# AlexGidiotis/Multimodal-Gesture-Recognition-with-LSTMs-and-CTC

Measured on AMD Instinct MI355X. Metric: train frames/sec, fusion BiLSTM+CTC, higher is better.
Workload: dtype f32

## Files before the change

multimodal-gesture-recognition-with-lstms-and-ctc_amd/csrc/gemm.hip:

```cpp
#include "common.h"
#include "split_f16.h"

namespace {

#ifndef MGR_GEMM_BK
#define MGR_GEMM_BK 16
#endif
#ifndef MGR_GEMM_NBUF
#define MGR_GEMM_NBUF 2
#endif
constexpr int BM = 128, BN = 128, BK = MGR_GEMM_BK, NBUF = MGR_GEMM_NBUF, LDS_LD = BM + 4;
constexpr int LPT = BK / 8;

struct RegTile {
  float v[4 * LPT];
};

__device__ __forceinline__ void load_kc(RegTile& r, const float* __restrict__ base, size_t ld, int m0, int k0, int Mlim,
                                        int Klim, bool vec, int tid) {
#pragma unroll
  for (int i = 0; i < LPT; ++i) {
    int idx4 = tid + i * 256;
    int m = idx4 / (BK / 4), k4 = (idx4 % (BK / 4)) * 4;
    int gm = m0 + m, gk = k0 + k4;
// ... 420 lines not shown
#pragma unroll
          for (int i = 0; i < APT; ++i) As[buf][ak & 3][ar + ARS * i][ak >> 2] = R.a[i];
        }
        *reinterpret_cast<float4*>(&Bs[buf][q][r][0]) = make_float4(R.w[0] * R.v[0], R.w[1] * R.v[1], R.w[2] * R.v[2], R.w[3] * R.v[3]);
      };
      auto mma = [&](int buf) {
        const int ra = wr * 64 + l31, ub = wc * 32 + l31;
        const f32x4 a00 = *reinterpret_cast<const f32x4*>(&As[buf][2 * lh][ra][0]);
        const f32x4 a01 = *reinterpret_cast<const f32x4*>(&As[buf][2 * lh + 1][ra][0]);
        const f32x4 a10 = *reinterpret_cast<const f32x4*>(&As[buf][2 * lh][ra + 32][0]);
        const f32x4 a11 = *reinterpret_cast<const f32x4*>(&As[buf][2 * lh + 1][ra + 32][0]);
        const f32x4 b0 = *reinterpret_cast<const f32x4*>(&Bs[buf][2 * lh][ub][0]);
        const f32x4 b1 = *reinterpret_cast<const f32x4*>(&Bs[buf][2 * lh + 1][ub][0]);
#pragma unroll
        for (int c = 0; c < 4; ++c) {
          acc[g][0] = __builtin_amdgcn_mfma_f32_32x32x2f32(a00[c], b0[c], acc[g][0], 0, 0, 0);
          acc[g][1] = __builtin_amdgcn_mfma_f32_32x32x2f32(a10[c], b0[c], acc[g][1], 0, 0, 0);
        }
#pragma unroll
        for (int c = 0; c < 4; ++c) {
          acc[g][0] = __builtin_amdgcn_mfma_f32_32x32x2f32(a01[c], b1[c], acc[g][0], 0, 0, 0);
          acc[g][1] = __builtin_amdgcn_mfma_f32_32x32x2f32(a11[c], b1[c], acc[g][1], 0, 0, 0);
        }
      };
      if (nst > 0) {
        Regs R0, R1;
        fetch(R0, 0);
        if (nst > 1) fetch(R1, 1);
        stash(R0, 0);
        __syncthreads();
        for (int st = 0; st < nst; st += 2) {
          if (st + 2 < nst) fetch(R0, st + 2);
          mma(0);
          if (st + 1 < nst) stash(R1, 1);
          __syncthreads();
          if (st + 1 < nst) {
            if (st + 3 < nst) fetch(R1, st + 3);
            mma(1);
            if (st + 2 < nst) stash(R0, 0);
            __syncthreads();
          }
        }
      }
    }
    const int unit = acc_col(u0 + wc * 32, l31);
    if (unit < H) {
      const float4 bias = *reinterpret_cast<const float4*>(bp + unit * 4);
      store_z_tile<true>(acc, 1.f, bias, Z, b, T, N, r0 + wr * 64, unit, lh);
    }
  }
}

constexpr int NP_MAXF = 64, NP_TU = 64, NP_RPW = 3;
static inline size_t np_lds_bytes(int F) { return ((size_t)SP_TM * (F | 1) + (size_t)4 * F * NP_TU) * sizeof(float); }

template <int XR>
__global__ __launch_bounds__(256, XR > 20 ? 1 : 2) void k_proj_narrow(const float* __restrict__ X, int ldx, const float* __restrict__ mask4,
                                                        const float* __restrict__ Wp, const float* __restrict__ bp, float* __restrict__ Z,
                                                        int B, int T, int F, int H) {
  constexpr int TM = SP_TM, TU = NP_TU;
  extern __shared__ __attribute__((aligned(16))) float np_lds[];
  __shared__ int Lf[4][NP_MAXF];
  __shared__ float Lv[4][NP_MAXF];
  __shared__ int Lc[4];
  const int pitch = F | 1;
  float* Xs = np_lds;
  float* Ws = np_lds + TM * pitch;
  const int tid = threadIdx.x, lane = tid & 63, wave = tid >> 6, wr = wave >> 1, wc = wave & 1;
  const int l31 = lane & 31, lh = lane >> 5;
  const int N = 4 * H;
  const int ncol = (H + TU - 1) / TU, nrow = (T + TM - 1) / TM, nchunk = (nrow + NP_RPW - 1) / NP_RPW;
  const XcdTile wt = xcd_tile(blockIdx.x, ncol);
  const int rc = wt.group;
  if (rc >= nchunk * B) return;
  const int u0 = wt.item * TU, b = rc / nchunk, rt0 = (rc % nchunk) * NP_RPW;
  const int rt1 = rt0 + NP_RPW < nrow ? rt0 + NP_RPW : nrow;
  {
    const int Fp = (F + SP_SK - 1) / SP_SK * SP_SK;
    const bool valid = lane < F;
    const float v = valid ? mask4[((size_t)wave * B + b) * F + lane] : 0.f;
    const bool kept = valid && v != 0.f;
    const unsigned long long kb = __ballot(kept), db = __ballot(valid && !kept), lower = (1ull << lane) - 1ull;
    const int cnt = __popcll(kb);
    if (valid) {
      const int pos = kept ? __popcll(kb & lower) : cnt + __popcll(db & lower);
      Lf[wave][pos] = lane;
      Lv[wave][pos] = v;
    } else if (lane < Fp) {
      Lf[wave][lane] = 0;
      Lv[wave][lane] = 0.f;
    }
    if (lane == 0) Lc[wave] = cnt;
  }
  {
    constexpr int WR = (XR + 1) / 2;
    float4 w[WR];
#pragma unroll
    for (int k = 0; k < WR; ++k) {
      const int i = tid + 256 * k < F * TU ? tid + 256 * k : F * TU - 1;
      const int f = i / TU, u = i % TU;
      const int uc = u0 + u < H ? u0 + u : H - 1;
      w[k] = *reinterpret_cast<const float4*>(Wp + (unsigned)((f * H + uc) * 4));
    }
#pragma unroll
    for (int k = 0; k < WR; ++k) {
      const int i = tid + 256 * k;
      if (i < F * TU) {
        const int f = i / TU, u = i % TU;
        Ws[(0 * F + f) * TU + u] = w[k].x;
        Ws[(1 * F + f) * TU + u] = w[k].y;
        Ws[(2 * F + f) * TU + u] = w[k].z;
        Ws[(3 * F + f) * TU + u] = w[k].w;
      }
    }
  }
  const int ra = wr * 64 + l31, ub = wc * 32 + l31;
  const int unit = u0 + ub;
  float4 bias = make_float4(0.f, 0.f, 0.f, 0.f);
  if (unit < H) bias = *reinterpret_cast<const float4*>(bp + unit * 4);
  const int dq = 256 / F, dr = 256 % F, row_0 = tid / F, col_0 = tid % F;
  const float* Xb = X + (size_t)b * T * ldx;
  float xv[XR];
  auto xload = [&](int rt) {
    int row = row_0, col = col_0;
#pragma unroll
    for (int k = 0; k < XR; ++k) {
      const int rw = row < TM ? row : TM - 1;
      const int rcl = rt * TM + rw < T ? rt * TM + rw : T - 1;
      xv[k] = Xb[(unsigned)(rcl * ldx + col)];
      row += dq;
      col += dr;
      if (col >= F) {
        col -= F;
        ++row;
      }
    }
  };
  xload(rt0);
  for (int rt = rt0; rt < rt1; ++rt) {
    const int r0 = rt * TM;
    __syncthreads();
    {
      int row = row_0, col = col_0;
#pragma unroll
      for (int k = 0; k < XR; ++k) {
        if (row < TM) Xs[row * pitch + col] = xv[k];
        row += dq;
        col += dr;
        if (col >= F) {
          col -= F;
          ++row;
        }
      }
    }
    __syncthreads();
    if (rt + 1 < rt1) xload(rt + 1);
    f32x16 acc[4][2];
    zero_acc(acc);
#pragma unroll
    for (int g = 0; g < 4; ++g) {
      const int nst = (Lc[g] + SP_SK - 1) / SP_SK;
      const float* Wsg = Ws + (size_t)g * F * TU + ub;
      const float* Xa = Xs + ra * pitch;
      for (int st = 0; st < nst; ++st) {
#pragma unroll
        for (int ks = 0; ks < 8; ++ks) {
          const int p = st * SP_SK + 2 * lh + (ks >> 2) + 4 * (ks & 3);
          const int f = Lf[g][p];
          const float bv = Wsg[f * TU] * Lv[g][p];
          acc[g][0] = __builtin_amdgcn_mfma_f32_32x32x2f32(Xa[f], bv, acc[g][0], 0, 0, 0);
          acc[g][1] = __builtin_amdgcn_mfma_f32_32x32x2f32(Xa[32 * pitch + f], bv, acc[g][1], 0, 0, 0);
        }
      }
    }
    if (unit < H) store_z_tile<true>(acc, 1.f, bias, Z, b, T, N, r0 + wr * 64, unit, lh);
  }
}

__global__ __launch_bounds__(256, 2) void k_gemm_nn_sparse16(const float* __restrict__ X, int ldx, const int* __restrict__ kidx,
                                                             const float* __restrict__ kval, const int* __restrict__ kcnt,
                                                             const float* __restrict__ Wp, const float* __restrict__ bp,
                                                             float* __restrict__ Z, int B, int T, int Fp, int F, int H,
                                                             const unsigned* __restrict__ wmax, float vmax, float sx, const unsigned* __restrict__ gate) {
  MGR_GATED(gate, false);
  constexpr int TM = SP_TM, TU = 64, SK = SP_SK, NT = 256, QT = 64, RPT = 2;
  __shared__ __attribute__((aligned(16))) _Float16 Ah[2][2][TM][8], Al[2][2][TM][8];
  __shared__ __attribute__((aligned(16))) _Float16 Bh[2][2][TU][8], Bl[2][2][TU][8];
  __shared__ unsigned short Ls[SP_MAXF];
  __shared__ float Vs[SP_MAXF];
  const int tid = threadIdx.x, lane = tid & 63, wave = tid >> 6, wr = wave >> 1, wc = wave & 1;
  const int N = 4 * H;
  const int q = tid / QT, r = tid % QT;
  const int l31 = lane & 31, lh = lane >> 5;
  const int ncol = (H + TU - 1) / TU, nrow = (T + TM - 1) / TM;
  const float sw = split_scale<SPLIT_NONFINITE_ZERO>(__uint_as_float(*wmax) * vmax, -60);
  const float inv = split_unscale(1.f, sw, sx);
  struct Regs {
    float a[RPT * 4], w[4], v[4];
  };
  const XcdTile wt = xcd_tile(blockIdx.x, ncol);
  const int rt = wt.group;
  if (rt >= nrow * B) return;
  const int u0 = wt.item * TU, r0 = (rt % nrow) * TM, b = rt / nrow;
  const float* Xb = X + (size_t)b * F * ldx + r0 + r;
  const int ucl = (u0 + r < H) ? u0 + r : H - 1;
  f32x16 acc[4][2];
  zero_acc(acc);
#pragma unroll
  for (int g = 0; g < 4; ++g) {
    const int nst1 = (kcnt[g * B + b] + SK - 1) / SK;
    const int nst = (nst1 + 1) & ~1;
    {
      const int* list = kidx + ((size_t)g * B + b) * Fp;
      const float* lval = kval + ((size_t)g * B + b) * Fp;
      for (int i = tid; i < nst * SK; i += NT) {
        const bool in = i < nst1 * SK;
        Ls[i] = in ? (unsigned short)list[i] : (unsigned short)0;
        Vs[i] = in ? lval[i] : 0.f;
      }
    }
    __syncthreads();
    const float* Wg = Wp + (size_t)g * F * H + ucl;
// ... 643 lines not shown
  const int Nd = 4 * H;
  const bool fast = (ldx % 4 == 0) && (F % BK == 0) && aligned16(X) && aligned16(Wp_fwd) && aligned16(Wp_rev);
  if (!fast || (2 * Nd + BN - 1) / BN >= 2 * ((Nd + BN - 1) / BN)) {
    int r = mgr_lstm_input_proj(c, X, ldx, mask4_fwd, Wp_fwd, bp_fwd, Z_fwd, B, T, F, H);
    if (r) return r;
    return mgr_lstm_input_proj(c, X, ldx, mask4_rev, Wp_rev, bp_rev, Z_rev, B, T, F, H);
  }
  dim3 grid((2 * Nd + BN - 1) / BN, (T + BM - 1) / BM, B);
  mgr_prof_begin(c, MGR_K_GEMM_NN);
  hipLaunchKernelGGL(k_gemm_nn2, grid, dim3(256), 0, mgr_stream(c), X, ldx, mask4_fwd, mask4_rev, Wp_fwd, Wp_rev, bp_fwd, bp_rev,
                     Z_fwd, Z_rev, B, T, F, Nd);
  MGR_LAUNCH_CHECK();
  mgr_prof_end(c, MGR_K_GEMM_NN);
  return 0;
}

static size_t sp_fp(int F) { return (size_t)(F + SP_SK - 1) / SP_SK * SP_SK; }

struct ProjDropWs { int* kidx; float* kval; int* kcnt; unsigned* wmax; float* Wg; size_t bytes; };
static ProjDropWs proj_dropout_ws_layout(void* ws, int B, int F, int H) {
  mgr_ws_carver w(ws);
  const size_t nl = (size_t)4 * B * sp_fp(F);
  return {w.take<int>(nl), w.take<float>(nl), w.take<int>((size_t)4 * B), w.take<unsigned>(64), w.take<float>((size_t)F * 4 * H), w.off};
}
size_t mgr_lstm_input_proj_dropout_ws_bytes(int B, int F, int H) { return proj_dropout_ws_layout(nullptr, B, F, H).bytes; }

static bool sparse_proj_shape(const mgr_ctx* c, float drop_rate, int F) {
  return drop_rate >= 0.3f && F >= 16 && F <= SP_MAXF && c->tune[MGR_TUNE_PROJ_DENSE] == 0;
}

int mgr_lstm_input_proj_dropout_wants_transposed(mgr_ctx* c, float drop_rate, int F) {
  return (c && sparse_proj_shape(c, drop_rate, F) && F >= 128) ? 1 : 0;
}

static int input_proj_dropout_impl(mgr_ctx* c, const float* X, int ldx, bool transposed, const float* mask4, float drop_rate,
                                   const float* Wp, const float* bp, float* Z, int B, int T, int F, int H, void* ws, size_t ws_bytes,
                                   float x_absmax = 0.f) {
  const int Fp = (int)sp_fp(F);
  const ProjDropWs L = proj_dropout_ws_layout(ws, B, F, H);
  int *kidx = L.kidx, *kcnt = L.kcnt;
  float *kval = L.kval, *Wg = L.Wg;
  unsigned* wmax = L.wmax;
  hipStream_t s = mgr_stream(c);
  const SplitCall sc = split_call(c, x_absmax, transposed && drop_rate < 0.99f, wmax + 1);
  const bool f16 = sc.f16;
  unsigned* const gate = sc.gate;
  const bool dense = f16 && (!mask4 || c->tune[MGR_TUNE_PROJ_DENSE16_MASKED] == 2);
  MGR_REQUIRE(mask4 || transposed, "a projection without a dropout mask is only handled from the transposed copy");
  const bool lists = !dense || gate;
  mgr_prof_begin(c, MGR_K_GEMM_NN);
  if (!transposed && mask4 && F >= 16 && F <= NP_MAXF && c->tune[MGR_TUNE_PROJ_WIDE_TILES] != 2) {
    if (!(c->attr_done & MGR_ATTR_PROJ_NARROW)) {
      MGR_HIP(hipFuncSetAttribute(reinterpret_cast<const void*>(k_proj_narrow<32>), hipFuncAttributeMaxDynamicSharedMemorySize, (int)np_lds_bytes(NP_MAXF)));
      c->attr_done |= MGR_ATTR_PROJ_NARROW;
    }
    const int nchunk = ((T + SP_TM - 1) / SP_TM + NP_RPW - 1) / NP_RPW;
    const int nwg = ((H + NP_TU - 1) / NP_TU) * ((nchunk * B + 7) / 8) * 8;
    if (F <= 20)
      hipLaunchKernelGGL(k_proj_narrow<10>, dim3(nwg), dim3(256), np_lds_bytes(F), s, X, ldx, mask4, Wp, bp, Z, B, T, F, H);
    else if (F <= 40)
      hipLaunchKernelGGL(k_proj_narrow<20>, dim3(nwg), dim3(256), np_lds_bytes(F), s, X, ldx, mask4, Wp, bp, Z, B, T, F, H);
    else
      hipLaunchKernelGGL(k_proj_narrow<32>, dim3(nwg), dim3(256), np_lds_bytes(F), s, X, ldx, mask4, Wp, bp, Z, B, T, F, H);
    MGR_LAUNCH_CHECK();
    mgr_prof_end(c, MGR_K_GEMM_NN);
    return 0;
  }
  if (lists && mask4)
    hipLaunchKernelGGL(k_mask_compact, dim3(4 * B), dim3(64), 0, s, mask4, F, Fp, kidx, kval, kcnt, (int*)nullptr, wmax);
  else if (lists)
    hipLaunchKernelGGL(k_mask_all, dim3(4 * B), dim3(64), 0, s, F, Fp, kidx, kval, kcnt, wmax);
  else
    MGR_HIP(hipMemsetAsync(wmax, 0, sizeof(unsigned), s));
  {
    const size_t n = (size_t)F * H;
    const int wgs = mgr_grid256(n, 2048);
    hipLaunchKernelGGL(k_gate_major, dim3(wgs), dim3(256), 0, s, Wp, Wg, F, H, wmax);
  }
  const bool wide = c->tune[MGR_TUNE_PROJ_WIDE_TILES] == 2 && !transposed;
  const int tu = wide ? 128 : 64;
  const int ntiles = ((H + tu - 1) / tu) * ((((T + SP_TM - 1) / SP_TM) * B + 7) / 8) * 8;
  if (f16) {
    const float sx = sc.sx;
    if (gate) {
      MGR_HIP(hipMemsetAsync(gate, 0, sizeof(unsigned), s));
      launch_absmax_gate(s, X, (size_t)B * F * ldx / 4, sc);
    }
    if (dense)
      hipLaunchKernelGGL(k_gemm_nn_dense16, dim3(ntiles), dim3(256), 0, s, X, ldx, mask4, Wg, bp, Z, B, T, F, H, wmax,
                         mask4 ? 1.f / (1.f - drop_rate) : 1.f, sx, gate);
    else
      hipLaunchKernelGGL(k_gemm_nn_sparse16, dim3(ntiles), dim3(256), 0, s, X, ldx, kidx, kval, kcnt, Wg, bp, Z, B, T, Fp, F, H, wmax,
                         1.f / (1.f - drop_rate), sx, gate);
    if (gate)
      hipLaunchKernelGGL((k_gemm_nn_sparse<2, true>), dim3(ntiles), dim3(256), 0, s, X, ldx, kidx, kval, kcnt, Wg, bp, Z, B, T, Fp, F, H, gate);
  } else if (transposed)
    hipLaunchKernelGGL((k_gemm_nn_sparse<2, true>), dim3(ntiles), dim3(256), 0, s, X, ldx, kidx, kval, kcnt, Wg, bp, Z, B, T, Fp, F, H, (const unsigned*)nullptr);
  else if (wide)
    hipLaunchKernelGGL((k_gemm_nn_sparse<4, false>), dim3(ntiles), dim3(512), 0, s, X, ldx, kidx, kval, kcnt, Wg, bp, Z, B, T, Fp, F, H, (const unsigned*)nullptr);
  else
    hipLaunchKernelGGL((k_gemm_nn_sparse<2, false>), dim3(ntiles), dim3(256), 0, s, X, ldx, kidx, kval, kcnt, Wg, bp, Z, B, T, Fp, F, H, (const unsigned*)nullptr);
  MGR_LAUNCH_CHECK();
  mgr_prof_end(c, MGR_K_GEMM_NN);
  return 0;
}

// ... 241 lines not shown
```

multimodal-gesture-recognition-with-lstms-and-ctc_amd/csrc/gemm_split.hip:

```cpp
#include "common.h"
#include "split_f16.h"

namespace {

typedef short tr4 __attribute__((__vector_size__(4 * sizeof(short))));
typedef short tr8 __attribute__((__vector_size__(8 * sizeof(short))));
typedef __attribute__((address_space(3))) char lds_char;
typedef __attribute__((address_space(3))) tr4 lds_tr4;

constexpr float XS_SCALE = 8192.f;
constexpr int PS_TM = 128, PS_SK = 32;
constexpr int PS_HP = 128;

__device__ __forceinline__ void ps_dma_b128(const void* gbase, unsigned voff, unsigned lds_addr) {
  unsigned keep;
  asm volatile("s_mov_b32 %0, m0\n\ts_mov_b32 m0, %3\n\ts_nop 0\n\tglobal_load_lds_dwordx4 %1, %2\n\ts_mov_b32 m0, %0"
               : "=&s"(keep)
               : "v"(voff), "s"(gbase), "s"(lds_addr)
               : "memory");
}
__device__ __forceinline__ int ps_swz(int row) { return ((row & 3) << 2) | ((row >> 2) & 3); }

__global__ __launch_bounds__(64) void k_lists32(const float* __restrict__ mask4, int F, int Fp32, int* __restrict__ lists, int* __restrict__ kcnt,
                                                int* __restrict__ kpos ,
// ... 338 lines not shown
}

constexpr int DW_BM = 128, DW_BN = 128, DW_TK = 32, DW_STAGE = 4 * 128 * 64;

__global__ __launch_bounds__(256) void k_rowmax_bt(const float* __restrict__ dZ, int N, int T, unsigned* __restrict__ zmax, float* __restrict__ zsum) {
  __shared__ float part[2][4][64];
  const int b = blockIdx.y, col = blockIdx.x * 64 + (threadIdx.x & 63), w = threadIdx.x >> 6;
  float m = 0.f, sm = 0.f;
  if (col < N) {
    const float* p = dZ + (size_t)b * T * N + col;
    for (int t = w; t < T; t += 4) {
      const float v = p[(size_t)t * N];
      m = fmaxf(m, fabsf(v));
      sm += v;
    }
  }
  part[0][w][threadIdx.x & 63] = m;
  part[1][w][threadIdx.x & 63] = sm;
  __syncthreads();
  if (w == 0 && col < N) {
    if (zmax) zmax[(size_t)b * N + col] = __float_as_uint(fmaxf(fmaxf(part[0][0][threadIdx.x], part[0][1][threadIdx.x]), fmaxf(part[0][2][threadIdx.x], part[0][3][threadIdx.x])));
    if (zsum) zsum[(size_t)b * N + col] = (part[1][0][threadIdx.x] + part[1][1][threadIdx.x]) + (part[1][2][threadIdx.x] + part[1][3][threadIdx.x]);
  }
}
__device__ __forceinline__ float dw_zscale(unsigned zm_bits) {
  return split_scale<SPLIT_NONFINITE_NAN>(__uint_as_float(zm_bits), -100);
}
__global__ __launch_bounds__(256) void k_transpose_split_scaled(const float* __restrict__ dZ, int N, float* __restrict__ dZS, int ldt, int T,
                                                                const unsigned* __restrict__ zmax, int vec) {
  const int b = blockIdx.z;
  ts_tile<true>(dZ + (size_t)b * T * N, N, dZS + (size_t)b * N * ldt, ldt, T, N, ldt, 0, zmax + (size_t)b * N, vec != 0);
}

typedef float dw_f4 __attribute__((ext_vector_type(4)));

template <int NW>
__global__ __launch_bounds__(64 * NW, 1) void k_dw_split(const char* __restrict__ XS, int ldt, const int* __restrict__ lists,
                                                         const int* __restrict__ kcnt, const unsigned* __restrict__ cword,
                                                         const char* __restrict__ dZS, const unsigned* __restrict__ zmax, float* __restrict__ P,
                                                         int B, int T, int Fp32, int F, int H) {
  constexpr int MB = 8 / NW;
  constexpr int NBUF = NW == 8 ? 4 : 3;
  constexpr int DPW = 16 / NW;
  extern __shared__ __attribute__((aligned(16))) char dw_smem[];
  const int tid = threadIdx.x, lane = tid & 63;
  const int wave = __builtin_amdgcn_readfirstlane(tid >> 6), wr = wave >> 1, wc = wave & 1;
  const int N = 4 * H;
  const int nft = (Fp32 + DW_BM - 1) / DW_BM, nut = (H + DW_BN - 1) / DW_BN, wps = 4 * nft * nut;
  const XcdTile wt = xcd_tile(blockIdx.x, wps);
  const int b = wt.group;
  if (b >= B) return;
  const int w_ = wt.item, g = w_ / (nft * nut), gb = g * B + b;
  const int q0 = ((w_ / nut) % nft) * DW_BM, u0 = (w_ % nut) * DW_BN;
  const int cnt = kcnt[gb];
  if (q0 >= cnt) return;
  const unsigned lds0 = (unsigned)(uintptr_t)(lds_char*)dw_smem;
  const char* XSb = XS + (size_t)b * F * ldt * 4;
  const char* ZSb = dZS + (size_t)b * N * ldt * 4;

  unsigned a_off[DPW], b_off[DPW];
#pragma unroll
  for (int i = 0; i < DPW; ++i) {
    const int id = DPW * wave + i, part = id >> 3, r = 16 * (id & 7) + (lane >> 2);
    const int ch = (lane & 3) ^ ((r >> 2) & 3);
    int q = q0 + r;
    q = q < cnt ? q : cnt - 1;
    const int f = lists[(size_t)gb * Fp32 + q] & 0xFFFF;
    a_off[i] = (unsigned)f * (unsigned)(4 * ldt) + (unsigned)(part * 2 * ldt + ch * 16);
    int u = u0 + r;
    u = u < H ? u : H - 1;
    b_off[i] = (unsigned)(4 * u + g) * (unsigned)(4 * ldt) + (unsigned)(part * 2 * ldt + ch * 16);
  }
  const int nst = (T + DW_TK - 1) / DW_TK;
  auto issue = [&](int n) {
    const unsigned buf = lds0 + (unsigned)(n % NBUF) * DW_STAGE;
    const int nn = (n < nst ? n : nst - 1) * DW_TK * 2;
#pragma unroll
    for (int i = 0; i < DPW; ++i) {
      ps_dma_b128(XSb + nn, a_off[i], buf + (unsigned)((DPW * wave + i) * 1024));
      ps_dma_b128(ZSb + nn, b_off[i], buf + (unsigned)(16384 + (DPW * wave + i) * 1024));
    }
  };
  const int l31 = lane & 31, kh = lane >> 5;
  unsigned oA[MB][2], oB[2][2];
#pragma unroll
  for (int mb = 0; mb < MB; ++mb) {
    const int m = 32 * MB * wr + 32 * mb + l31;
#pragma unroll
    for (int ks = 0; ks < 2; ++ks) oA[mb][ks] = (unsigned)(m * 64 + 16 * ((2 * ks + kh) ^ ((m >> 2) & 3)));
  }
#pragma unroll
  for (int nb = 0; nb < 2; ++nb) {
    const int nn = 64 * wc + 32 * nb + l31;
#pragma unroll
    for (int ks = 0; ks < 2; ++ks) oB[nb][ks] = (unsigned)(16384 + nn * 64 + 16 * ((2 * ks + kh) ^ ((nn >> 2) & 3)));
  }
  f32x16 acc[MB][2];
  zero_acc(acc);
  constexpr int PD = NBUF - 1;
#pragma unroll
  for (int s0 = 0; s0 < PD; ++s0) issue(s0);
  for (int n = 0; n < nst; ++n) {
    if constexpr (NW == 8)
      asm volatile("s_waitcnt vmcnt(8)" ::: "memory");
    else
      asm volatile("s_waitcnt vmcnt(8)" ::: "memory");
    __syncthreads();
    issue(n + PD);
    const unsigned sb = lds0 + (unsigned)(n % NBUF) * DW_STAGE;
#pragma unroll
    for (int ks = 0; ks < 2; ++ks) {
      dw_f4 fa[MB][2], fb[2][2];
      const unsigned ca0 = sb + oA[0][ks], ca1 = sb + oA[MB - 1][ks], cb0 = sb + oB[0][ks], cb1 = sb + oB[1][ks];
      if constexpr (MB == 1)
        asm volatile("ds_read_b128 %0, %6\n\tds_read_b128 %2, %7\n\tds_read_b128 %4, %8\n\tds_read_b128 %1, %6 offset:8192"
                     "\n\tds_read_b128 %3, %7 offset:8192\n\tds_read_b128 %5, %8 offset:8192\n\ts_waitcnt lgkmcnt(0)"
                     : "=&v"(fa[0][0]), "=&v"(fa[0][1]), "=&v"(fb[0][0]), "=&v"(fb[0][1]), "=&v"(fb[1][0]), "=&v"(fb[1][1])
                     : "v"(ca0), "v"(cb0), "v"(cb1)
                     : "memory");
      else
        asm volatile("ds_read_b128 %0, %8\n\tds_read_b128 %4, %10\n\tds_read_b128 %6, %11\n\tds_read_b128 %2, %9"
                     "\n\tds_read_b128 %1, %8 offset:8192\n\tds_read_b128 %5, %10 offset:8192\n\tds_read_b128 %7, %11 offset:8192"
                     "\n\tds_read_b128 %3, %9 offset:8192\n\ts_waitcnt lgkmcnt(0)"
                     : "=&v"(fa[0][0]), "=&v"(fa[0][1]), "=&v"(fa[MB - 1][0]), "=&v"(fa[MB - 1][1]), "=&v"(fb[0][0]), "=&v"(fb[0][1]),
                       "=&v"(fb[1][0]), "=&v"(fb[1][1])
                     : "v"(ca0), "v"(ca1), "v"(cb0), "v"(cb1)
                     : "memory");
#pragma unroll
      for (int mb = 0; mb < MB; ++mb) {
        const f16x8 ah = __builtin_bit_cast(f16x8, fa[mb][0]), al = __builtin_bit_cast(f16x8, fa[mb][1]);
#pragma unroll
        for (int nb = 0; nb < 2; ++nb) {
          const f16x8 bh = __builtin_bit_cast(f16x8, fb[nb][0]), bl = __builtin_bit_cast(f16x8, fb[nb][1]);
          mfma3_split(ah, al, bh, bl, acc[mb][nb]);
        }
      }
    }
  }
  asm volatile("s_waitcnt vmcnt(0)" ::: "memory");
  const float cf = __uint_as_float(*cword) * (1.f / XS_SCALE);
  float* out = P + (size_t)gb * Fp32 * H;
#pragma unroll
  for (int nb = 0; nb < 2; ++nb) {
    const int u = acc_col(u0 + 64 * wc + 32 * nb, l31);
    const float cz = u < H ? 1.f / dw_zscale(zmax[(size_t)b * N + 4 * u + g]) : 0.f;
#pragma unroll
    for (int mb = 0; mb < MB; ++mb)
#pragma unroll
      for (int reg = 0; reg < 16; ++reg) {
        const int r = acc_row(32 * MB * wr + 32 * mb, reg, kh);
        if (q0 + r < cnt && u < H) out[(size_t)(q0 + r) * H + u] = acc[mb][nb][reg] * cf * cz;
      }
  }
}

constexpr int DG_SB = 8;
__global__ __launch_bounds__(256) void k_dw_gather32(const float* __restrict__ P, const int* __restrict__ kpos, float* __restrict__ dWp, int B, int F,
                                                     int Fp32, int H, int vec ) {
  const size_t n = (size_t)F * H;
  for (size_t i = blockIdx.x * (size_t)256 + threadIdx.x; i < n; i += (size_t)gridDim.x * 256) {
    const int u = (int)(i % H);
    const int f = (int)(i / H);
    float sacc[4] = {0.f, 0.f, 0.f, 0.f};
    for (int b0 = 0; b0 < B; b0 += DG_SB) {
      int pos[DG_SB][4];
      float v[DG_SB][4];
#pragma unroll
      for (int k = 0; k < DG_SB; ++k)
#pragma unroll
        for (int g = 0; g < 4; ++g) pos[k][g] = b0 + k < B ? (kpos ? kpos[((size_t)g * B + b0 + k) * F + f] : f) : -1;
#pragma unroll
      for (int k = 0; k < DG_SB; ++k)
#pragma unroll
        for (int g = 0; g < 4; ++g) {
          v[k][g] = 0.f;
          if (pos[k][g] >= 0) v[k][g] = P[(((size_t)g * B + b0 + k) * Fp32 + pos[k][g]) * H + u];
        }
#pragma unroll
      for (int k = 0; k < DG_SB; ++k)
#pragma unroll
        for (int g = 0; g < 4; ++g)
          if (pos[k][g] >= 0) sacc[g] += v[k][g];
    }
    float* out = dWp + ((size_t)f * H + u) * 4;
    if (vec) {
      *reinterpret_cast<float4*>(out) = make_float4(sacc[0], sacc[1], sacc[2], sacc[3]);
    } else {
#pragma unroll
      for (int g = 0; g < 4; ++g) out[g] = sacc[g];
    }
  }
}

static bool aligned16(const void* p) { return (reinterpret_cast<uintptr_t>(p) & 15) == 0; }
static int hp_of(int H) { return (H + PS_HP - 1) / PS_HP * PS_HP; }
static int fp32_of(int F) { return (F + PS_SK - 1) / PS_SK * PS_SK; }

}

extern "C" {

struct ProjTsWs { int *lists, *kcnt; unsigned* words ; _Float16* WSp; int* kpos; size_t bytes; };
static ProjTsWs proj_ts_ws_layout(const void* ws, int B, int F, int H) {
  mgr_ws_carver w(ws);
  return {w.take<int>((size_t)4 * B * fp32_of(F)), w.take<int>((size_t)4 * B), w.take<unsigned>(64),
          w.take<_Float16>((size_t)4 * (F + 1) * 2 * hp_of(H)), w.take<int>((size_t)4 * B * F), w.off};
}
size_t mgr_lstm_input_proj_dropout_ts_ws_bytes(int B, int F, int H) { return proj_ts_ws_layout(nullptr, B, F, H).bytes; }

int mgr_lstm_input_proj_dropout_ts(mgr_ctx* c, const float* XS, int ldt, const float* mask4, float drop_rate, const float* Wp,
                                   const float* bp, float* Z, int B, int T, int F, int H, void* ws, size_t ws_bytes) {
  MGR_REQUIRE(c && XS && Wp && bp && Z, "null argument");
  MGR_REQUIRE(B > 0 && T > 0 && H > 0 && F >= 16 && F <= 2048, "bad shape (16 <= F <= 2048)");
  MGR_REQUIRE(ldt % PS_TM == 0 && ldt >= T, "the split copy must be padded to whole row tiles of %d (ldt %d, T %d)", PS_TM, ldt, T);
  MGR_REQUIRE(aligned16(XS) && aligned16(bp) && aligned16(Z) && aligned16(Wp), "XS / bp / Z / Wp must be 16-byte aligned");
  MGR_REQUIRE((size_t)F * ldt * 4 < (1ull << 32), "sample block too large");
  const ProjTsWs L = proj_ts_ws_layout(ws, B, F, H);
  const size_t need = L.bytes;
  MGR_REQUIRE(ws && ws_bytes >= need, "workspace too small");
  (void)drop_rate;
  const int Fp32 = fp32_of(F), Hp = hp_of(H);
  int *lists = L.lists, *kcnt = L.kcnt, *kpos = L.kpos;
  unsigned* words = L.words;
  _Float16* WSp = L.WSp;
  hipStream_t s = mgr_stream(c);
  if (!(c->attr_done & MGR_ATTR_PROJ_SPLIT)) {
    MGR_HIP(hipFuncSetAttribute(reinterpret_cast<const void*>(k_proj_split<2>), hipFuncAttributeMaxDynamicSharedMemorySize, PsCfg<2>::LDS));
    MGR_HIP(hipFuncSetAttribute(reinterpret_cast<const void*>(k_proj_split<4>), hipFuncAttributeMaxDynamicSharedMemorySize, PsCfg<4>::LDS));
    c->attr_done |= MGR_ATTR_PROJ_SPLIT;
  }
  mgr_prof_begin(c, MGR_K_GEMM_NN);
  const char* region = reinterpret_cast<const char*>(words);
  const size_t region_bytes = (size_t)(reinterpret_cast<const char*>(kpos) - region);
  bool frozen = false;
  int hit = -1;
  for (int i = 0; i < MGR_MAX_FROZEN; ++i) frozen = frozen || (c->frozen_w[i] == Wp);
  if (frozen) {
    for (int i = 0; i < MGR_MAX_FROZEN; ++i) {
      const mgr_ctx::PlaneEntry& e = c->planes[i];
      if (e.Wp == Wp && e.ws == ws && e.B == B && e.F == F && e.H == H) hit = i;
    }
  }
// ... 36 lines not shown
  return {w.take<int>(nl), w.take<int>((size_t)4 * B), w.take<unsigned>(64), w.take<int>((size_t)4 * B * F), w.take<float>(nl * H)};
}
struct DwTsWs { DwTsGroup dW; float* dZS; unsigned* zmax; DwTsGroup dU; size_t bytes; };
static DwTsWs dw_ts_ws_layout(void* ws, int B, int T, int F, int H, int ldt) {
  mgr_ws_carver w(ws, mgr_lstm_param_grads_ws_bytes(B, T, F, H));
  return {dw_ts_group(w, B, F, H), w.take<float>((size_t)B * 4 * H * ldt), w.take<unsigned>((size_t)B * 4 * H), dw_ts_group(w, B, H, H), w.off};
}
size_t mgr_lstm_param_grads_dropout_ts_ws_bytes(int B, int T, int F, int H, int ldt) { return dw_ts_ws_layout(nullptr, B, T, F, H, ldt).bytes; }

int mgr_lstm_param_grads_dropout_ts(mgr_ctx* c, const float* XS, int ldt, const float* mask4, float drop_rate, const float* Hs, int ldh,
                                    const float* dZ, float* dWp, float* dUp, float* dbp, int B, int T, int F, int H, int reverse,
                                    void* ws, size_t ws_bytes, const unsigned* dzmax, const float* dbsum, const void* proj_ws,
                                    const float* HsT) {
  MGR_REQUIRE(c && XS && mask4 && Hs && dZ && dWp && dUp && dbp, "null argument");
  mgr_planes_forget_range(c, ws, ws_bytes);
  MGR_REQUIRE(B > 0 && T > 0 && H > 0 && F >= 16 && F <= 2048 && ldh >= H, "bad shape (16 <= F <= 2048)");
  MGR_REQUIRE(ldt % 32 == 0 && ldt >= (T + DW_TK - 1) / DW_TK * DW_TK, "the split copy must be padded to whole stages of %d time steps (ldt %d, T %d)", DW_TK, ldt, T);
  MGR_REQUIRE(aligned16(dZ) && aligned16(XS), "dZ / XS must be 16-byte aligned");
  MGR_REQUIRE((size_t)F * ldt * 4 < (1ull << 32) && (size_t)4 * H * ldt * 4 < (1ull << 32), "sample block too large");
  const DwTsWs L = dw_ts_ws_layout(ws, B, T, F, H, ldt);
  MGR_REQUIRE(ws && ws_bytes >= L.bytes, "workspace too small");
  (void)drop_rate;
  mgr_prof_begin(c, MGR_K_GEMM_TN);
  MGR_REQUIRE(!HsT || (H >= 16 && aligned16(HsT) && (size_t)H * ldt * 4 < (1ull << 32)), "HsT: 16 <= H, 16-byte aligned");
  int r = mgr_param_grads_du_db(c, Hs, ldh, dZ, HsT ? nullptr : dUp, dbp, B, T, F, H, reverse, ws, dbsum);
  if (r) return r;
  const int Fp32 = fp32_of(F), N = 4 * H;
  int *lists = L.dW.lists, *kcnt = L.dW.kcnt, *kpos = L.dW.kpos;
  unsigned* words = L.dW.words;
  float *P = L.dW.P, *dZS = L.dZS;
  const unsigned* zmax = dzmax ? dzmax : L.zmax;
  const int Hp32 = fp32_of(H);
  int *lists2 = L.dU.lists, *kcnt2 = L.dU.kcnt;
  unsigned* words2 = L.dU.words;
  float* P2 = L.dU.P;
  hipStream_t s = mgr_stream(c);
  if (!(c->attr_done & MGR_ATTR_DW_SPLIT)) {
    MGR_HIP(hipFuncSetAttribute(reinterpret_cast<const void*>(k_dw_split<8>), hipFuncAttributeMaxDynamicSharedMemorySize, 4 * DW_STAGE));
    MGR_HIP(hipFuncSetAttribute(reinterpret_cast<const void*>(k_dw_split<4>), hipFuncAttributeMaxDynamicSharedMemorySize, 3 * DW_STAGE));
    c->attr_done |= MGR_ATTR_DW_SPLIT;
  }
  if (proj_ws) {
    const ProjTsWs Lp = proj_ts_ws_layout(proj_ws, B, F, H);
    lists = Lp.lists, kcnt = Lp.kcnt, words = Lp.words, kpos = Lp.kpos;
  } else {
    MGR_HIP(hipMemsetAsync(words, 0, 2 * sizeof(unsigned), s));
    hipLaunchKernelGGL(k_lists32, dim3(4 * B), dim3(64), 0, s, mask4, F, Fp32, lists, kcnt, kpos, words + 1);
  }
  if (!dzmax) hipLaunchKernelGGL(k_rowmax_bt, dim3((N + 63) / 64, B), dim3(256), 0, s, dZ, N, T, const_cast<unsigned*>(zmax), (float*)nullptr);
  hipLaunchKernelGGL(k_transpose_split_scaled, dim3((ldt + TS_TT - 1) / TS_TT, (N + 63) / 64, B), dim3(256), 0, s, dZ, N, dZS, ldt, T, zmax,
                     (int)(ldt % 8 == 0));
  if (HsT) {
    const int grid2 = 8 * ((B + 7) / 8) * 4 * ((Hp32 + DW_BM - 1) / DW_BM) * ((H + DW_BN - 1) / DW_BN);
    MGR_HIP(hipMemsetAsync(words2, 0, 2 * sizeof(unsigned), s));
    hipLaunchKernelGGL(k_lists32, dim3(4 * B), dim3(64), 0, s, (const float*)nullptr, H, Hp32, lists2, kcnt2, (int*)nullptr, words2 + 1);
    if (c->tune[MGR_TUNE_PROJ_TS_TILE] == 1)
      hipLaunchKernelGGL(k_dw_split<4>, dim3(grid2), dim3(256), 3 * DW_STAGE, s, reinterpret_cast<const char*>(HsT), ldt, lists2, kcnt2, words2 + 1,
                         reinterpret_cast<const char*>(dZS), zmax, P2, B, T, Hp32, H, H);
    else
      hipLaunchKernelGGL(k_dw_split<8>, dim3(grid2), dim3(512), 4 * DW_STAGE, s, reinterpret_cast<const char*>(HsT), ldt, lists2, kcnt2, words2 + 1,
                         reinterpret_cast<const char*>(dZS), zmax, P2, B, T, Hp32, H, H);
    const size_t n2 = (size_t)H * H;
    hipLaunchKernelGGL(k_dw_gather32, dim3(mgr_grid256(n2, 4096)), dim3(256), 0, s, P2, (const int*)nullptr, dUp, B, H,
                       Hp32, H, (int)aligned16(dUp));
  }
  const int grid = 8 * ((B + 7) / 8) * 4 * ((Fp32 + DW_BM - 1) / DW_BM) * ((H + DW_BN - 1) / DW_BN);
  if (c->tune[MGR_TUNE_PROJ_TS_TILE] == 1)
    hipLaunchKernelGGL(k_dw_split<4>, dim3(grid), dim3(256), 3 * DW_STAGE, s, reinterpret_cast<const char*>(XS), ldt, lists, kcnt, words + 1,
                       reinterpret_cast<const char*>(dZS), zmax, P, B, T, Fp32, F, H);
  else
    hipLaunchKernelGGL(k_dw_split<8>, dim3(grid), dim3(512), 4 * DW_STAGE, s, reinterpret_cast<const char*>(XS), ldt, lists, kcnt, words + 1,
                       reinterpret_cast<const char*>(dZS), zmax, P, B, T, Fp32, F, H);
  const size_t n = (size_t)F * H;
  hipLaunchKernelGGL(k_dw_gather32, dim3(mgr_grid256(n, 4096)), dim3(256), 0, s, P, kpos, dWp, B, F, Fp32, H,
                     (int)aligned16(dWp));
  MGR_LAUNCH_CHECK();
  mgr_prof_end(c, MGR_K_GEMM_TN);
  return 0;
}

int mgr_weight_planes_cache(mgr_ctx* c, const float* Wp, int frozen) {
  MGR_REQUIRE(c && Wp, "null argument");
  for (int i = 0; i < MGR_MAX_FROZEN; ++i) {
    if (c->planes[i].Wp == Wp) c->planes[i] = mgr_ctx::PlaneEntry{};
    if (c->frozen_w[i] == Wp) c->frozen_w[i] = nullptr;
  }
  if (!frozen) return 0;
  for (int i = 0; i < MGR_MAX_FROZEN; ++i)
    if (!c->frozen_w[i]) {
      c->frozen_w[i] = Wp;
      return 0;
    }
  const int victim = (int)(c->frozen_evict++ % MGR_MAX_FROZEN);
  for (int i = 0; i < MGR_MAX_FROZEN; ++i)
    if (c->planes[i].Wp == c->frozen_w[victim]) c->planes[i] = mgr_ctx::PlaneEntry{};
  c->frozen_w[victim] = Wp;
  return 0;
}

int mgr_transpose_bt_split(mgr_ctx* c, const float* X, int ldx, float* XS, int ldt, int B, int T, int F) {
  MGR_REQUIRE(c && X && XS, "null argument");
  MGR_REQUIRE(B > 0 && T > 0 && F > 0 && ldx >= F && ldt >= T && ldt % 8 == 0, "bad shape");
  mgr_prof_begin(c, MGR_K_MISC);
  hipLaunchKernelGGL(k_transpose_split, dim3((ldt + TS_TT - 1) / TS_TT, (F + 63) / 64, B), dim3(256), 0, mgr_stream(c), X, ldx, XS, ldt, T, F, 0LL, ldt, 0,
                     (int)aligned16(XS));
  MGR_LAUNCH_CHECK();
  mgr_prof_end(c, MGR_K_MISC);
  return 0;
}

int mgr_transpose_bt_split_shift(mgr_ctx* c, const float* X, int ldx, float* XS, int ldt, int B, int T, int F, int tshift) {
  MGR_REQUIRE(c && X && XS, "null argument");
  MGR_REQUIRE(B > 0 && T > 0 && F > 0 && ldx >= F && ldt >= T && ldt % 8 == 0 && tshift >= -1 && tshift <= 1, "bad shape");
  mgr_prof_begin(c, MGR_K_MISC);
  hipLaunchKernelGGL(k_transpose_split, dim3((ldt + TS_TT - 1) / TS_TT, (F + 63) / 64, B), dim3(256), 0, mgr_stream(c), X, ldx, XS, ldt, T, F, 0LL, ldt, tshift,
                     (int)aligned16(XS));
  MGR_LAUNCH_CHECK();
  mgr_prof_end(c, MGR_K_MISC);
  return 0;
}

}

int mgr_rowmax_bt(mgr_ctx* c, const float* dZ, int N, int T, int B, unsigned* zmax, float* zsum) {
  hipLaunchKernelGGL(k_rowmax_bt, dim3((N + 63) / 64, B), dim3(256), 0, mgr_stream(c), dZ, N, T, zmax, zsum);
  MGR_LAUNCH_CHECK();
  return 0;
// ... 9 lines not shown
```

Baseline: 8.360 million.

## Pre-permute masked weights in narrow projection and skip list building for dense dW

The narrow projection kernel now writes weights into LDS already permuted into kept-feature order and pre-multiplied by the dropout mask value. This removes an indirect lookup and a multiply from the inner MFMA loop, at the cost of a barrier and scattered LDS writes during staging. The recurrent dW path no longer builds identity index lists with a memset and an extra kernel; it passes null lists and treats them as the identity. The gather kernel is templated to split gates across threads and to prefetch positions for the next batch block, exposing more parallelism when there are few gates.

```diff
diff --git a/multimodal-gesture-recognition-with-lstms-and-ctc_amd/csrc/gemm.hip b/multimodal-gesture-recognition-with-lstms-and-ctc_amd/csrc/gemm.hip
--- a/multimodal-gesture-recognition-with-lstms-and-ctc_amd/csrc/gemm.hip
+++ b/multimodal-gesture-recognition-with-lstms-and-ctc_amd/csrc/gemm.hip
@@ -496,7 +496,8 @@
 }
 
 constexpr int NP_MAXF = 64, NP_TU = 64, NP_RPW = 3;
-static inline size_t np_lds_bytes(int F) { return ((size_t)SP_TM * (F | 1) + (size_t)4 * F * NP_TU) * sizeof(float); }
+static inline int np_fp(int F) { return (F + SP_SK - 1) / SP_SK * SP_SK; }
+static inline size_t np_lds_bytes(int F) { return ((size_t)SP_TM * (F | 1) + (size_t)4 * np_fp(F) * NP_TU) * sizeof(float); }
 
 template <int XR>
 __global__ __launch_bounds__(256, XR > 20 ? 1 : 2) void k_proj_narrow(const float* __restrict__ X, int ldx, const float* __restrict__ mask4,
@@ -505,9 +506,10 @@
   constexpr int TM = SP_TM, TU = NP_TU;
   extern __shared__ __attribute__((aligned(16))) float np_lds[];
   __shared__ int Lf[4][NP_MAXF];
+  __shared__ int Lp[4][NP_MAXF];
   __shared__ float Lv[4][NP_MAXF];
   __shared__ int Lc[4];
-  const int pitch = F | 1;
+  const int pitch = F | 1, Fp = (F + SP_SK - 1) / SP_SK * SP_SK;
   float* Xs = np_lds;
   float* Ws = np_lds + TM * pitch;
   const int tid = threadIdx.x, lane = tid & 63, wave = tid >> 6, wr = wave >> 1, wc = wave & 1;
@@ -520,7 +522,6 @@
   const int u0 = wt.item * TU, b = rc / nchunk, rt0 = (rc % nchunk) * NP_RPW;
   const int rt1 = rt0 + NP_RPW < nrow ? rt0 + NP_RPW : nrow;
   {
-    const int Fp = (F + SP_SK - 1) / SP_SK * SP_SK;
     const bool valid = lane < F;
     const float v = valid ? mask4[((size_t)wave * B + b) * F + lane] : 0.f;
     const bool kept = valid && v != 0.f;
@@ -529,10 +530,10 @@
     if (valid) {
       const int pos = kept ? __popcll(kb & lower) : cnt + __popcll(db & lower);
       Lf[wave][pos] = lane;
-      Lv[wave][pos] = v;
+      Lp[wave][lane] = pos;
+      Lv[wave][lane] = v;
     } else if (lane < Fp) {
       Lf[wave][lane] = 0;
-      Lv[wave][lane] = 0.f;
     }
     if (lane == 0) Lc[wave] = cnt;
   }
@@ -546,15 +547,19 @@
       const int uc = u0 + u < H ? u0 + u : H - 1;
       w[k] = *reinterpret_cast<const float4*>(Wp + (unsigned)((f * H + uc) * 4));
     }
+    __syncthreads();
 #pragma unroll
     for (int k = 0; k < WR; ++k) {
       const int i = tid + 256 * k;
       if (i < F * TU) {
         const int f = i / TU, u = i % TU;
-        Ws[(0 * F + f) * TU + u] = w[k].x;
-        Ws[(1 * F + f) * TU + u] = w[k].y;
-        Ws[(2 * F + f) * TU + u] = w[k].z;
-        Ws[(3 * F + f) * TU + u] = w[k].w;
+        const float wg[4] = {w[k].x, w[k].y, w[k].z, w[k].w};
+#pragma unroll
+        for (int g = 0; g < 4; ++g) Ws[(g * Fp + Lp[g][f]) * TU + u] = wg[g] * Lv[g][f];
+        if (f == 0)
+          for (int p = F; p < Fp; ++p)
+#pragma unroll
+            for (int g = 0; g < 4; ++g) Ws[(g * Fp + p) * TU + u] = wg[g] * 0.f;
       }
     }
   }
@@ -604,14 +609,14 @@
 #pragma unroll
     for (int g = 0; g < 4; ++g) {
       const int nst = (Lc[g] + SP_SK - 1) / SP_SK;
-      const float* Wsg = Ws + (size_t)g * F * TU + ub;
+      const float* Wsg = Ws + (size_t)g * Fp * TU + ub;
       const float* Xa = Xs + ra * pitch;
       for (int st = 0; st < nst; ++st) {
 #pragma unroll
         for (int ks = 0; ks < 8; ++ks) {
           const int p = st * SP_SK + 2 * lh + (ks >> 2) + 4 * (ks & 3);
           const int f = Lf[g][p];
-          const float bv = Wsg[f * TU] * Lv[g][p];
+          const float bv = Wsg[p * TU];
           acc[g][0] = __builtin_amdgcn_mfma_f32_32x32x2f32(Xa[f], bv, acc[g][0], 0, 0, 0);
           acc[g][1] = __builtin_amdgcn_mfma_f32_32x32x2f32(Xa[32 * pitch + f], bv, acc[g][1], 0, 0, 0);
         }
@@ -1361,6 +1366,7 @@
   if (!transposed && mask4 && F >= 16 && F <= NP_MAXF && c->tune[MGR_TUNE_PROJ_WIDE_TILES] != 2) {
     if (!(c->attr_done & MGR_ATTR_PROJ_NARROW)) {
       MGR_HIP(hipFuncSetAttribute(reinterpret_cast<const void*>(k_proj_narrow<32>), hipFuncAttributeMaxDynamicSharedMemorySize, (int)np_lds_bytes(NP_MAXF)));
+      MGR_HIP(hipFuncSetAttribute(reinterpret_cast<const void*>(k_proj_narrow<20>), hipFuncAttributeMaxDynamicSharedMemorySize, (int)np_lds_bytes(40)));
       c->attr_done |= MGR_ATTR_PROJ_NARROW;
     }
     const int nchunk = ((T + SP_TM - 1) / SP_TM + NP_RPW - 1) / NP_RPW;
diff --git a/multimodal-gesture-recognition-with-lstms-and-ctc_amd/csrc/gemm_split.hip b/multimodal-gesture-recognition-with-lstms-and-ctc_amd/csrc/gemm_split.hip
--- a/multimodal-gesture-recognition-with-lstms-and-ctc_amd/csrc/gemm_split.hip
+++ b/multimodal-gesture-recognition-with-lstms-and-ctc_amd/csrc/gemm_split.hip
@@ -414,7 +414,7 @@
   if (b >= B) return;
   const int w_ = wt.item, g = w_ / (nft * nut), gb = g * B + b;
   const int q0 = ((w_ / nut) % nft) * DW_BM, u0 = (w_ % nut) * DW_BN;
-  const int cnt = kcnt[gb];
+  const int cnt = lists ? kcnt[gb] : F;
   if (q0 >= cnt) return;
   const unsigned lds0 = (unsigned)(uintptr_t)(lds_char*)dw_smem;
   const char* XSb = XS + (size_t)b * F * ldt * 4;
@@ -427,7 +427,7 @@
     const int ch = (lane & 3) ^ ((r >> 2) & 3);
     int q = q0 + r;
     q = q < cnt ? q : cnt - 1;
-    const int f = lists[(size_t)gb * Fp32 + q] & 0xFFFF;
+    const int f = lists ? lists[(size_t)gb * Fp32 + q] & 0xFFFF : q;
     a_off[i] = (unsigned)f * (unsigned)(4 * ldt) + (unsigned)(part * 2 * ldt + ch * 16);
     int u = u0 + r;
     u = u < H ? u : H - 1;
@@ -500,7 +500,7 @@
     }
   }
   asm volatile("s_waitcnt vmcnt(0)" ::: "memory");
-  const float cf = __uint_as_float(*cword) * (1.f / XS_SCALE);
+  const float cf = (lists ? __uint_as_float(*cword) : 1.f) * (1.f / XS_SCALE);
   float* out = P + (size_t)gb * Fp32 * H;
 #pragma unroll
   for (int nb = 0; nb < 2; ++nb) {
@@ -516,40 +516,59 @@
   }
 }
 
-constexpr int DG_SB = 8;
+template <int NG, int SB, bool POS >
 __global__ __launch_bounds__(256) void k_dw_gather32(const float* __restrict__ P, const int* __restrict__ kpos, float* __restrict__ dWp, int B, int F,
                                                      int Fp32, int H, int vec ) {
-  const size_t n = (size_t)F * H;
-  for (size_t i = blockIdx.x * (size_t)256 + threadIdx.x; i < n; i += (size_t)gridDim.x * 256) {
+  const size_t n = (size_t)F * H, nt = n * (4 / NG);
+  const size_t pstride = (size_t)Fp32 * H;
+  for (size_t j = blockIdx.x * (size_t)256 + threadIdx.x; j < nt; j += (size_t)gridDim.x * 256) {
+    const size_t i = j % n;
+    const int g0 = (int)(j / n) * NG;
     const int u = (int)(i % H);
     const int f = (int)(i / H);
-    float sacc[4] = {0.f, 0.f, 0.f, 0.f};
-    for (int b0 = 0; b0 < B; b0 += DG_SB) {
-      int pos[DG_SB][4];
-      float v[DG_SB][4];
-#pragma unroll
-      for (int k = 0; k < DG_SB; ++k)
-#pragma unroll
-        for (int g = 0; g < 4; ++g) pos[k][g] = b0 + k < B ? (kpos ? kpos[((size_t)g * B + b0 + k) * F + f] : f) : -1;
-#pragma unroll
-      for (int k = 0; k < DG_SB; ++k)
-#pragma unroll
-        for (int g = 0; g < 4; ++g) {
-          v[k][g] = 0.f;
-          if (pos[k][g] >= 0) v[k][g] = P[(((size_t)g * B + b0 + k) * Fp32 + pos[k][g]) * H + u];
+    float sacc[NG];
+    int pos[SB][NG];
+#pragma unroll
+    for (int g = 0; g < NG; ++g) sacc[g] = 0.f;
+#pragma unroll
+    for (int k = 0; k < SB; ++k)
+#pragma unroll
+      for (int g = 0; g < NG; ++g) {
+        const int q = POS ? kpos[((size_t)(g0 + g) * B + (k < B ? k : B - 1)) * F + f] : f;
+        pos[k][g] = k < B ? q : -1;
+      }
+    for (int b0 = 0; b0 < B; b0 += SB) {
+      float v[SB][NG];
+#pragma unroll
+      for (int k = 0; k < SB; ++k)
+#pragma unroll
+        for (int g = 0; g < NG; ++g) {
+          const size_t at = ((size_t)(g0 + g) * B + b0 + k) * pstride + (size_t)pos[k][g] * H + u;
+          v[k][g] = P[pos[k][g] >= 0 ? at : (size_t)0];
         }
-#pragma unroll
-      for (int k = 0; k < DG_SB; ++k)
-#pragma unroll
-        for (int g = 0; g < 4; ++g)
-          if (pos[k][g] >= 0) sacc[g] += v[k][g];
-    }
-    float* out = dWp + ((size_t)f * H + u) * 4;
-    if (vec) {
-      *reinterpret_cast<float4*>(out) = make_float4(sacc[0], sacc[1], sacc[2], sacc[3]);
+      int nxt[SB][NG];
+#pragma unroll
+      for (int k = 0; k < SB; ++k)
+#pragma unroll
+        for (int g = 0; g < NG; ++g) {
+          const int bn = b0 + SB + k;
+          const int q = POS ? kpos[((size_t)(g0 + g) * B + (bn < B ? bn : B - 1)) * F + f] : f;
+          nxt[k][g] = bn < B ? q : -1;
+        }
+#pragma unroll
+      for (int k = 0; k < SB; ++k)
+#pragma unroll
+        for (int g = 0; g < NG; ++g) {
+          sacc[g] = pos[k][g] >= 0 ? sacc[g] + v[k][g] : sacc[g];
+          pos[k][g] = nxt[k][g];
+        }
+    }
+    float* out = dWp + ((size_t)f * H + u) * 4 + g0;
+    if (NG == 4 && vec) {
+      *reinterpret_cast<float4*>(out) = make_float4(sacc[0], sacc[NG > 1 ? 1 : 0], sacc[NG > 2 ? 2 : 0], sacc[NG > 3 ? 3 : 0]);
     } else {
 #pragma unroll
-      for (int g = 0; g < 4; ++g) out[g] = sacc[g];
+      for (int g = 0; g < NG; ++g) out[g] = sacc[g];
     }
   }
 }
@@ -692,16 +711,14 @@
                      (int)(ldt % 8 == 0));
   if (HsT) {
     const int grid2 = 8 * ((B + 7) / 8) * 4 * ((Hp32 + DW_BM - 1) / DW_BM) * ((H + DW_BN - 1) / DW_BN);
-    MGR_HIP(hipMemsetAsync(words2, 0, 2 * sizeof(unsigned), s));
-    hipLaunchKernelGGL(k_lists32, dim3(4 * B), dim3(64), 0, s, (const float*)nullptr, H, Hp32, lists2, kcnt2, (int*)nullptr, words2 + 1);
     if (c->tune[MGR_TUNE_PROJ_TS_TILE] == 1)
-      hipLaunchKernelGGL(k_dw_split<4>, dim3(grid2), dim3(256), 3 * DW_STAGE, s, reinterpret_cast<const char*>(HsT), ldt, lists2, kcnt2, words2 + 1,
+      hipLaunchKernelGGL(k_dw_split<4>, dim3(grid2), dim3(256), 3 * DW_STAGE, s, reinterpret_cast<const char*>(HsT), ldt, (const int*)nullptr, (const int*)nullptr, (const unsigned*)nullptr,
                          reinterpret_cast<const char*>(dZS), zmax, P2, B, T, Hp32, H, H);
     else
-      hipLaunchKernelGGL(k_dw_split<8>, dim3(grid2), dim3(512), 4 * DW_STAGE, s, reinterpret_cast<const char*>(HsT), ldt, lists2, kcnt2, words2 + 1,
+      hipLaunchKernelGGL(k_dw_split<8>, dim3(grid2), dim3(512), 4 * DW_STAGE, s, reinterpret_cast<const char*>(HsT), ldt, (const int*)nullptr, (const int*)nullptr, (const unsigned*)nullptr,
                          reinterpret_cast<const char*>(dZS), zmax, P2, B, T, Hp32, H, H);
     const size_t n2 = (size_t)H * H;
-    hipLaunchKernelGGL(k_dw_gather32, dim3(mgr_grid256(n2, 4096)), dim3(256), 0, s, P2, (const int*)nullptr, dUp, B, H,
+    hipLaunchKernelGGL((k_dw_gather32<1, 32, false>), dim3(mgr_grid256(4 * n2, 4096)), dim3(256), 0, s, P2, (const int*)nullptr, dUp, B, H,
                        Hp32, H, (int)aligned16(dUp));
   }
   const int grid = 8 * ((B + 7) / 8) * 4 * ((Fp32 + DW_BM - 1) / DW_BM) * ((H + DW_BN - 1) / DW_BN);
@@ -712,7 +729,7 @@
     hipLaunchKernelGGL(k_dw_split<8>, dim3(grid), dim3(512), 4 * DW_STAGE, s, reinterpret_cast<const char*>(XS), ldt, lists, kcnt, words + 1,
                        reinterpret_cast<const char*>(dZS), zmax, P, B, T, Fp32, F, H);
   const size_t n = (size_t)F * H;
-  hipLaunchKernelGGL(k_dw_gather32, dim3(mgr_grid256(n, 4096)), dim3(256), 0, s, P, kpos, dWp, B, F, Fp32, H,
+  hipLaunchKernelGGL((k_dw_gather32<4, 8, true>), dim3(mgr_grid256(n, 4096)), dim3(256), 0, s, P, kpos, dWp, B, F, Fp32, H,
                      (int)aligned16(dWp));
   MGR_LAUNCH_CHECK();
   mgr_prof_end(c, MGR_K_GEMM_TN);
```

Measured after the change: 8.364 million (median of 6 runs). No clear change (+0.0%).
